# svenstaro/bvh

Hardware: AMD Instinct MI355X
Metric: Mrays/s (build+traverse) (higher is better)
Workload: dtype f32; 1 GPU; configs[1]: create_n_cubes(10000), 120000 triangles f32/3D, 1000000 create_ray rays per GPU; step = build_par+flatten+traverse; triangles=120000, rays_per_gpu=1000000, rays_total=1000000, scene_dist=single, flat_array=eager, parallelism=rays sharded x1

## Files before the change

bvh_amd/csrc/build.hip:

```cpp
#include "flatten_node.hpp"

namespace bvhgpu {

constexpr int MAXLV = 96;
constexpr int CTR_SMALL = 0;
constexpr int CTR_MID2 = 2;
constexpr int CTR_FLAGS = 4;
constexpr int CTR_TOPMASK = BUILD_CTR_TOPMASK;
constexpr uint32_t BUILD_FLAG_NONFINITE = 1u;
constexpr uint32_t BUILD_FLAG_PERSIST_GAVE_UP = BSTAT_UNFINISHED;
constexpr uint32_t BUILD_FLAG_EMPTY_SPLIT = 2u;
#ifndef BVH_MID_SMALL_MAXN
#define BVH_MID_SMALL_MAXN 768
#endif
#ifndef BVH_MID_SMALL_THREADS
#define BVH_MID_SMALL_THREADS 384
#endif
template <typename T> struct MidSmallScene {
    static constexpr int MAXN = BVH_MID_SMALL_MAXN;
    static constexpr int THREADS = BVH_MID_SMALL_THREADS;
    static constexpr int HANDOFF = SMALL_MAX;
};
#ifndef BVH_MID_LARGE_MAXN
#define BVH_MID_LARGE_MAXN 1536
#endif
#ifndef BVH_MID_LARGE_THREADS
#define BVH_MID_LARGE_THREADS 256
#endif
template <typename T> struct MidLargeScene {
    static constexpr int MAXN = sizeof(T) == 4 ? BVH_MID_LARGE_MAXN : BVH_MID_LARGE_MAXN * 2 / 3;
    static constexpr int THREADS = BVH_MID_LARGE_THREADS;
    static constexpr int HANDOFF = SMALL_MAX;
};
constexpr size_t MID_SCENE_SPLIT = 250000;
#ifndef BVH_STAT_REP
#define BVH_STAT_REP 8
#endif
constexpr int STAT_REP = BVH_STAT_REP;
constexpr int CTR_LEVEL0 = 16;
constexpr int CTR_XDIR = CTR_LEVEL0 + 2 * MAXLV;
static_assert((CTR_XDIR + 8 * 4) * 4 <= 1024, "the directory lives inside the counter page");
constexpr size_t ROOTKEY_OFF = 1024;
constexpr int PREP_MAX_WG = 1024;

__host__ __device__ inline int lvl_slot(int L) { return L < MAXLV - 2 ? L : (MAXLV - 2 + (L & 1)); }

template <typename T> struct ItemStats {
    typename Traits<T>::Key k[NUM_BUCKETS * STAT_KEYS];
    uint32_t cnt[NUM_BUCKETS];
    uint32_t _pad[2];
};

template <typename T> struct LevelArgs {
    Item<T>* item[2];
    uint4* tile_map[3];
    ItemStats<T>* stats[3];
    uint32_t* tile_cnt[3];
    uint8_t* bk[2];
    uint32_t slot_div, n_slots, n_tiles;
};

template <typename T> struct BuildArgs {
    LevelArgs<T> lv;
    uint32_t mid_max;
    const T* aabbs;
    const T* src;
    typename Traits<T>::Node* nodes;
    uint32_t* node_start;
    uint32_t* node_count;
    uint32_t* shape_node;
    uint16_t* node_slot;
    uint32_t* slot_entry;
    uint32_t n_slots;
    uint32_t* wslot_node;
    uint32_t* idx[2];
    uint8_t* bk;
    Item<T>* big[2];
    Item<T>* mid2;
    Item<T>* small;
    ItemStats<T>* stats[2];
    uint32_t* tile_item[2];
    uint32_t* tile_cnt;
    uint32_t* chunk_cnt[2];
    uint32_t n_chunks;
    FlattenArgs<T> fl;
    uint32_t fl_parts;
    uint32_t tile2;
    uint32_t* ctr;
    typename Traits<T>::Key* rootkeys;
    uint32_t prep_wgs;
    uint32_t n;
    unsigned long long* xbar;
};
constexpr int XBAR_WORDS = 8 * 32;

__device__ __forceinline__ bool key_is_min(int j) { return j < 3 || (j >= 6 && j < 9); }

template <typename T>
__device__ void push_item(const BuildArgs<T>& a, int next_level, uint32_t ni, uint32_t parent, uint32_t start,
                          uint32_t count, const T* A, const T* C, uint32_t heap, int lane);
template <typename T> __device__ void init_stats(ItemStats<T>* s, int lane);

template <typename T> __global__ __launch_bounds__(256) void k_prep(BuildArgs<T> a) {
    using Tr = Traits<T>;
    using Key = typename Tr::Key;
    __shared__ Key sk[STAT_KEYS];
    if (threadIdx.x < STAT_KEYS) sk[threadIdx.x] = key_is_min(threadIdx.x) ? Tr::KEY_POS_INF : Tr::KEY_NEG_INF;
    __syncthreads();
    T loc[STAT_KEYS];
#pragma unroll
    for (int j = 0; j < STAT_KEYS; j++) loc[j] = key_is_min(j) ? Tr::inf() : -Tr::inf();
    if (a.lv.tile_map[0]) {
        const uint32_t gt = blockIdx.x * blockDim.x + threadIdx.x, gs = gridDim.x * blockDim.x;
        for (uint32_t i = gt; i < 3u * a.lv.n_tiles; i += gs) a.lv.tile_map[i / a.lv.n_tiles][i % a.lv.n_tiles] = make_uint4(NONE, 0u, 0u, 0u);
        const uint32_t nc = a.lv.n_tiles * (uint32_t)NUM_BUCKETS;
        for (uint32_t i = gt; i < 3u * nc; i += gs) a.lv.tile_cnt[i / nc][i % nc] = 0u;
    }
    if (a.lv.tile_map[0] && blockIdx.x == 0 && threadIdx.x < WAVE)
        for (int r = 0; r < STAT_REP; r++) init_stats<T>(&a.lv.stats[0][r], (int)threadIdx.x);
    if (a.xbar && blockIdx.x == 0)
        for (uint32_t i = threadIdx.x; i < (uint32_t)XBAR_WORDS; i += blockDim.x) a.xbar[i] = 0ull;
    if (a.chunk_cnt[0] && blockIdx.x == 1 % gridDim.x)
        for (uint32_t i = threadIdx.x; i < 2u * a.n_chunks * 2u * (uint32_t)NUM_BUCKETS; i += blockDim.x) a.chunk_cnt[0][i] = 0u;
    if (blockIdx.x == 0) {
        for (uint32_t i = threadIdx.x; i < a.n_slots; i += blockDim.x) a.slot_entry[i] = NONE;
        for (uint32_t i = threadIdx.x; i < WIDE_SLOTS; i += blockDim.x) a.wslot_node[i] = NONE;
    }
    const bool copy = a.src != a.aabbs;
    T* own = const_cast<T*>(a.aabbs);
    bool bad = false;
    for (uint32_t i = blockIdx.x * blockDim.x + threadIdx.x; i < a.n; i += gridDim.x * blockDim.x) {
        a.idx[0][i] = i;
        const T* b = a.src + 6 * (size_t)i;
        T bx[6];
#pragma unroll
        for (int k = 0; k < 6; k++) bx[k] = b[k];
#pragma unroll
        for (int k = 0; k < 6; k++) bad = bad || !(fabs(bx[k]) < Tr::inf());
        if (copy) {
#pragma unroll
            for (int k = 0; k < 6; k++) own[6 * (size_t)i + k] = bx[k];
        }
#pragma unroll
        for (int k = 0; k < 3; k++) {
            const T c = center1(bx[k], bx[3 + k]);
            loc[k] = join_min(loc[k], bx[k]);
            loc[3 + k] = join_max(loc[3 + k], bx[3 + k]);
            loc[6 + k] = join_min(loc[6 + k], c);
            loc[9 + k] = join_max(loc[9 + k], c);
        }
    }
    {
        const int lane = lane_id();
#pragma unroll
        for (int d = 32; d > 0; d >>= 1) {
            T u[STAT_KEYS];
#pragma unroll
            for (int j = 0; j < STAT_KEYS; j++) u[j] = lane_fetch(loc[j], (lane ^ d) << 2);
#pragma unroll
            for (int j = 0; j < STAT_KEYS; j++) loc[j] = key_is_min(j) ? join_min(loc[j], u[j]) : join_max(loc[j], u[j]);
        }
        if (lane == 0) {
#pragma unroll
            for (int j = 0; j < STAT_KEYS; j++) {
                if (key_is_min(j)) atomicMin(&sk[j], Tr::key(loc[j]));
                else atomicMax(&sk[j], Tr::key(loc[j]));
            }
        }
    }
    if (a.n > 1 && __any(bad) && lane_id() == 0) atomicOr(&a.ctr[CTR_FLAGS], BUILD_FLAG_NONFINITE);
    __syncthreads();
    if (threadIdx.x < STAT_KEYS) a.rootkeys[(size_t)blockIdx.x * STAT_KEYS + threadIdx.x] = sk[threadIdx.x];
}

template <typename T> __global__ __launch_bounds__(256) void k_root(BuildArgs<T> a, uint32_t prep_wgs, int fused) {
    using Tr = Traits<T>;
    using Key = typename Tr::Key;
    __shared__ Key sk[STAT_KEYS];
    if (threadIdx.x < STAT_KEYS) sk[threadIdx.x] = key_is_min(threadIdx.x) ? Tr::KEY_POS_INF : Tr::KEY_NEG_INF;
    __syncthreads();
    for (uint32_t e = threadIdx.x; e < prep_wgs * (uint32_t)STAT_KEYS; e += blockDim.x) {
        const Key v = a.rootkeys[e];
        const int j = (int)(e % (uint32_t)STAT_KEYS);
        if (key_is_min(j)) atomicMin(&sk[j], v);
        else atomicMax(&sk[j], v);
    }
    __syncthreads();
    if (threadIdx.x < WAVE) {
        T A[6], C[6];
#pragma unroll
        for (int k = 0; k < 6; k++) { A[k] = Tr::unkey(sk[k]); C[k] = Tr::unkey(sk[6 + k]); }
        uint32_t flags = a.ctr[CTR_FLAGS];
        if (a.n > 1) {
            bool ovf = false;
#pragma unroll
            for (int k = 0; k < 3; k++) ovf = ovf || !(fabs(C[3 + k] - C[k]) < Tr::inf());
            if (ovf) { flags |= BUILD_FLAG_NONFINITE; if (threadIdx.x == 0) atomicOr(&a.ctr[CTR_FLAGS], BUILD_FLAG_NONFINITE); }
        }
        if (flags & BUILD_FLAG_NONFINITE) return;
        if (fused && a.n > a.mid_max) {
            const int lane = (int)threadIdx.x;
            Item<T>* it = &a.lv.item[0][0];
            if (lane == 0) {
                it->ni = 0; it->parent = 0; it->start = 0; it->count = a.n; it->tile_base = 0; it->parity = 0; it->heap = 1u; it->_r1 = 0;
                a.ctr[CTR_LEVEL0] = 1u;
            }
            if (lane < 6) { it->A[lane] = A[lane]; it->C[lane] = C[lane]; }
            const uint32_t ntile = (a.n + TILE - 1) / TILE;
            for (uint32_t j = lane; j < ntile; j += WAVE) a.lv.tile_map[0][j] = make_uint4(0u, 0u, a.n, 0u);
            for (int r = 0; r < STAT_REP; r++) init_stats<T>(&a.lv.stats[0][r], lane);
        } else {
            push_item<T>(a, 0, 0u, 0u, 0u, a.n, A, C, 1u, (int)threadIdx.x);
        }
    }
}

template <typename T> __device__ void init_stats(ItemStats<T>* s, int lane) {
    using Tr = Traits<T>;
    for (int j = lane; j < NUM_BUCKETS * STAT_KEYS; j += WAVE)
        s->k[j] = key_is_min(j % STAT_KEYS) ? Tr::KEY_POS_INF : Tr::KEY_NEG_INF;
    if (lane < NUM_BUCKETS) s->cnt[lane] = 0;
}

template <typename T>
__device__ void push_item(const BuildArgs<T>& a, int next_level, uint32_t ni, uint32_t parent, uint32_t start,
                          uint32_t count, const T* A, const T* C, uint32_t heap, int lane) {
    const int nslot = lvl_slot(next_level);
    const int npar = next_level & 1;
    uint32_t slot = 0, tb = 0;
    const bool is_small = count <= (uint32_t)SMALL_MAX;
    const bool is_mid2 = !is_small && count <= a.mid_max;
    const uint32_t ntile = (count + a.tile2 - 1) / a.tile2;
// ... 497 lines not shown
#pragma unroll
        for (int k = 0; k < 6; k++) { la[k] = Tr::unkey(scratch[sp * 6 + k]); ra[k] = Tr::unkey(scratch[36 + (sp + 1) * 6 + k]); }
        const T sa_parent = surface_area(A);
        const T cl = (T)ln * surface_area(la);
        const T cr = (T)(total - ln) * surface_area(ra);
        const T num = cl + cr;
        cost = num / sa_parent;
    }
    T min_cost = Tr::inf();
    int best = -1;
#pragma unroll
    for (int sp = 0; sp < NUM_BUCKETS - 1; sp++) {
        const T c = lane_bcast_rt(cost, sp);
        const bool take = degen ? (sp == 0) : (c < min_cost);
        if (take) { min_cost = c; best = sp; }
    }
    uint32_t nl = 0;
#pragma unroll
    for (int b = 0; b < NUM_BUCKETS; b++) nl += (best < 0 ? b == 0 : b <= best) ? cnt[b] : 0u;
    if (lane < 6) {
        const int k = lane;
        const bool mn = k < 3;
        T al, ar, cl, cr;
        if (best < 0) {
            al = ar = cl = cr = mn ? Tr::inf() : -Tr::inf();
        } else {
            Key kl = mn ? Tr::KEY_POS_INF : Tr::KEY_NEG_INF, kr = kl;
#pragma unroll
            for (int b = 0; b < NUM_BUCKETS; b++) {
                const Key x = stk[b * STAT_KEYS + 6 + k];
                const Key jl = mn ? (x < kl ? x : kl) : (x > kl ? x : kl);
                const Key jr = mn ? (x < kr ? x : kr) : (x > kr ? x : kr);
                kl = b <= best ? jl : kl;
                kr = b <= best ? kr : jr;
            }
            al = Tr::unkey(scratch[best * 6 + k]);
            ar = Tr::unkey(scratch[36 + (best + 1) * 6 + k]);
            cl = Tr::unkey(kl); cr = Tr::unkey(kr);
        }
        out->AL[k] = al; out->AR[k] = ar; out->CL[k] = cl; out->CR[k] = cr;
    }
    if (lane == 0) { out->nl = nl; out->no_winner = best < 0 ? 1u : 0u; }
    __builtin_amdgcn_fence(__ATOMIC_RELEASE, "wavefront");
    __builtin_amdgcn_wave_barrier();
    __builtin_amdgcn_fence(__ATOMIC_ACQUIRE, "wavefront");
}

template <typename T> struct LevelChild {
    uint32_t start, count, kind, slot, tile0, ax, degen, half;
    T cmin, ext;
};
constexpr int LEVEL_TGT = 4;

template <typename T> __device__ __forceinline__ void level_child_derive(LevelChild<T>* c, const T* C, uint32_t start, uint32_t count,
                                                                          uint32_t mid_max, uint32_t slot_div) {
    c->start = start; c->count = count;
    c->kind = count <= (uint32_t)SMALL_MAX ? 0u : (count <= mid_max ? 1u : 3u);
    c->slot = start / slot_div;
    c->tile0 = start / (uint32_t)TILE + c->slot;
    const int ax = largest_axis(C);
    c->ax = (uint32_t)ax;
    c->cmin = C[ax];
    c->ext = C[3 + ax] - C[ax];
    c->degen = (c->ext < Traits<T>::eps()) ? 1u : 0u;
    c->half = count / 2;
}

#ifdef BVH_LEVEL_PROFILE
__device__ unsigned long long g_level_prof[2 * 8 * 1024];
#define LEVEL_STAMP(i) do { if ((L == BVH_LEVEL_PROFILE || L == BVH_LEVEL_PROFILE + 1) && threadIdx.x == 0 && blockIdx.x < 1024) \
        g_level_prof[8 * (blockIdx.x + 1024 * (L - BVH_LEVEL_PROFILE)) + (i)] = wall_clock64(); } while (0)
#else
#define LEVEL_STAMP(i) do { } while (0)
#endif
__device__ __forceinline__ uint32_t wave_sum_u32(uint32_t x) {
    int v = (int)x;
    v += __builtin_amdgcn_update_dpp(0, v, 0x111, 0xF, 0xF, true);
    v += __builtin_amdgcn_update_dpp(0, v, 0x112, 0xF, 0xF, true);
    v += __builtin_amdgcn_update_dpp(0, v, 0x114, 0xF, 0xF, true);
    v += __builtin_amdgcn_update_dpp(0, v, 0x118, 0xF, 0xF, true);
    return (uint32_t)(__builtin_amdgcn_readlane(v, 15) + __builtin_amdgcn_readlane(v, 31) + __builtin_amdgcn_readlane(v, 47) +
                      __builtin_amdgcn_readlane(v, 63));
}
constexpr int LEVEL_TC_REP = 4;
constexpr int LEVEL_PT = TILE / 256;

#ifndef BVH_LEVEL_THREADS
#define BVH_LEVEL_THREADS 256
#endif
#ifndef BVH_LEVEL_EARLY_DUTIES
#define BVH_LEVEL_EARLY_DUTIES 1
#endif
constexpr int LEVEL_THREADS = BVH_LEVEL_THREADS;
constexpr bool LEVEL_DEDICATED = LEVEL_THREADS > 256;
constexpr unsigned long long XCD_SPIN_TICKS = 200000ull;
template <typename T, bool ROOT, bool DEV = false> __global__ __launch_bounds__(LEVEL_THREADS) void k_level(BuildArgs<T> a, int L_first) {
    using Tr = Traits<T>;
    using Key = typename Tr::Key;
    static_assert(TILE % 256 == 0 && LEVEL_PT >= 1 && LEVEL_PT <= 4, "a tile is a whole number of 256-thread rounds");
    static_assert(!(ROOT && DEV), "the root is binned by a launch of its own");
    const LevelArgs<T>& v = a.lv;
    uint32_t wg_rank = blockIdx.x, wg_count = gridDim.x, g0 = 0u, g1 = v.n_tiles, s0 = 0u, s1 = v.n_slots;
    __shared__ uint32_t s_live, s_go;
    __shared__ unsigned long long s_word;
    uint32_t live_seen = 0;
    if constexpr (DEV) {
        const uint32_t grp = blockIdx.x & 7u;
        wg_rank = blockIdx.x >> 3; wg_count = gridDim.x >> 3;
        const uint32_t* xd = &a.ctr[CTR_XDIR + 4 * grp];
        const uint32_t kind = xd[0], start = xd[2], count = xd[3];
        if (kind != 3u || (a.ctr[CTR_FLAGS] & BUILD_FLAG_NONFINITE)) return;
        const uint32_t sd = v.slot_div, end = start + count;
        g0 = start / (uint32_t)TILE + start / sd; g1 = end / (uint32_t)TILE + end / sd;
        s0 = start / sd; s1 = end / sd;
    }
    uint32_t* const live = &s_live;
  for (int L = L_first, round = 0; ; L++, round++) {
    if constexpr (DEV) {
        if (threadIdx.x == 0) s_live = 0u;
        __syncthreads();
    }
    const int bP = (L + 2) % 3, bC = L % 3, bN = (L + 1) % 3;
    const uint32_t* src = ROOT ? a.idx[0] : a.idx[(L + 1) & 1];
    uint32_t* dst = a.idx[L & 1];
    const uint8_t* bk_src = v.bk[(L + 1) & 1];
    uint8_t* bk_dst = v.bk[L & 1];
    const int lane = lane_id(), w = threadIdx.x >> 6;
    const bool shaper = !LEVEL_DEDICATED || w > 0;
    const int sw = LEVEL_DEDICATED ? w - 1 : w;
    const uint32_t stid = LEVEL_DEDICATED ? threadIdx.x - 64u : threadIdx.x;
    const unsigned long long lt = lanemask_lt();
    LEVEL_STAMP(0);
    uint4 tm_first = make_uint4(NONE, 0u, 0u, 0u);
    if (!ROOT && g0 + wg_rank < g1) tm_first = ldx4<DEV>(&v.tile_map[bP][g0 + wg_rank]);
    __shared__ Key s_rootk[STAT_KEYS];
    if (ROOT) {
        if (threadIdx.x < STAT_KEYS) s_rootk[threadIdx.x] = key_is_min(threadIdx.x) ? Tr::KEY_POS_INF : Tr::KEY_NEG_INF;
        __syncthreads();
        for (uint32_t e = threadIdx.x; e < a.prep_wgs * (uint32_t)STAT_KEYS; e += LEVEL_THREADS) {
            const Key x = a.rootkeys[e];
            const int j = (int)(e % (uint32_t)STAT_KEYS);
            if (key_is_min(j)) atomicMin(&s_rootk[j], x);
            else atomicMax(&s_rootk[j], x);
        }
        __syncthreads();
        bool bad = (a.ctr[CTR_FLAGS] & BUILD_FLAG_NONFINITE) != 0u;
#pragma unroll
        for (int k = 0; k < 3; k++) bad = bad || !(fabs(Tr::unkey(s_rootk[9 + k]) - Tr::unkey(s_rootk[6 + k])) < Tr::inf());
        if (bad) {
            if (blockIdx.x == 0 && threadIdx.x == 0) atomicOr(&a.ctr[CTR_FLAGS], BUILD_FLAG_NONFINITE);
            return;
        }
        const uint32_t root_tiles = (a.n + TILE - 1) / TILE;
        if (blockIdx.x == 0) {
            Item<T>* it = &v.item[0][0];
            if (threadIdx.x == 0) {
                it->ni = 0; it->parent = 0; it->start = 0; it->count = a.n; it->tile_base = 0; it->parity = 0; it->heap = 1u; it->_r1 = 0;
                a.ctr[CTR_LEVEL0] = 1u;
            }
            if (threadIdx.x < 6) { it->A[threadIdx.x] = Tr::unkey(s_rootk[threadIdx.x]); it->C[threadIdx.x] = Tr::unkey(s_rootk[6 + threadIdx.x]); }
            for (uint32_t j = threadIdx.x; j < root_tiles; j += LEVEL_THREADS) v.tile_map[0][j] = make_uint4(0u, 0u, a.n, 0u);
        }
        if (blockIdx.x < root_tiles) tm_first = make_uint4(0u, 0u, a.n, 0u);
    }

    {
        const uint32_t gt = wg_rank * (uint32_t)LEVEL_THREADS + threadIdx.x, gs = wg_count * (uint32_t)LEVEL_THREADS;
        for (uint32_t i = g0 + gt; i < g1; i += gs) {
            if constexpr (DEV) stx<true>(&v.tile_map[bN][i].x, NONE);
            else v.tile_map[bN][i] = make_uint4(NONE, 0u, 0u, 0u);
        }
        for (uint32_t i = g0 * (uint32_t)NUM_BUCKETS + gt; i < g1 * (uint32_t)NUM_BUCKETS; i += gs) stx<DEV>(&v.tile_cnt[bN][i], 0u);
        constexpr uint32_t NK = NUM_BUCKETS * STAT_KEYS;
        const uint32_t e0 = s0 * (uint32_t)STAT_REP, e1 = s1 * (uint32_t)STAT_REP;
        for (uint32_t i = e0 * NK + gt; i < e1 * NK; i += gs) {
            const uint32_t e = i / NK, j = i % NK;
            stx<DEV>(&v.stats[bN][e].k[j], key_is_min((int)(j % STAT_KEYS)) ? Tr::KEY_POS_INF : Tr::KEY_NEG_INF);
        }
        for (uint32_t i = e0 * (uint32_t)NUM_BUCKETS + gt; i < e1 * (uint32_t)NUM_BUCKETS; i += gs) stx<DEV>(&v.stats[bN][i / NUM_BUCKETS].cnt[i % NUM_BUCKETS], 0u);
    }

    __shared__ Key sk[2][BIN_REP][NUM_BUCKETS * STAT_KEYS];
    __shared__ uint32_t sc[2][BIN_REP][NUM_BUCKETS];
    __shared__ uint32_t tcnt[LEVEL_TC_REP][NUM_BUCKETS][LEVEL_TGT][NUM_BUCKETS];
    __shared__ uint32_t run0[NUM_BUCKETS], wsum[4][NUM_BUCKETS], wcnt[4][LEVEL_PT][NUM_BUCKETS];
    __shared__ LevelChild<T> ch[2];
    __shared__ LevelSel<T> sel;
    __shared__ ItemStats<T> s_merged;
    __shared__ Key s_sah[72];
    const int rp = (int)(stid & (BIN_REP - 1)), rt = (int)(stid & (LEVEL_TC_REP - 1));

    for (uint32_t g = g0 + wg_rank; g < g1; g += wg_count) {
        const uint4 tm = g == g0 + wg_rank ? tm_first : (ROOT ? make_uint4(g < (a.n + TILE - 1) / TILE ? 0u : NONE, 0u, a.n, 0u) : ldx4<DEV>(&v.tile_map[bP][g]));
        const uint32_t slotP = tm.x;
        if (slotP == NONE) continue;
        LEVEL_STAMP(1);
        const uint32_t start = tm.y, count = tm.z;
        const Item<T>* P = &v.item[ROOT ? 0 : ((L + 1) & 1)][slotP];
        const uint32_t tile0P = start / (uint32_t)TILE + slotP;
        const uint32_t tl = g - tile0P, ntl = (count + TILE - 1) / TILE;
        const uint32_t p0 = start + tl * TILE;
        const uint32_t pend = min(start + count, p0 + (uint32_t)TILE);

        Key rk[2][STAT_REP];
        uint32_t rc[STAT_REP];
        T PA[6], PC[6];
        uint32_t P_ni = 0, P_heap = 0, P_parent = 0;
        if (!ROOT && w == 0) {
            const ItemStats<T>* rep = &v.stats[bP][(size_t)slotP * STAT_REP];
#pragma unroll
            for (int h = 0; h < 2; h++) {
                const int j = lane + 64 * h;
#pragma unroll
                for (int r = 0; r < STAT_REP; r++) rk[h][r] = j < NUM_BUCKETS * STAT_KEYS ? ldx<DEV>(&rep[r].k[j]) : (Key)0;
            }
#pragma unroll
            for (int r = 0; r < STAT_REP; r++) rc[r] = lane < NUM_BUCKETS ? ldx<DEV>(&rep[r].cnt[lane]) : 0u;
#pragma unroll
            for (int k = 0; k < 6; k++) { PA[k] = ldx<DEV>(&P->A[k]); PC[k] = ldx<DEV>(&P->C[k]); }
            if (tl == 0) { P_ni = ldx<DEV>(&P->ni); P_heap = ldx<DEV>(&P->heap); P_parent = ldx<DEV>(&P->parent); }
        }
        uint32_t sh[LEVEL_PT];
        int bo[LEVEL_PT];
        T bx[LEVEL_PT][6];
#pragma unroll
        for (int u = 0; u < LEVEL_PT; u++) {
            const uint32_t p = p0 + (uint32_t)u * 256u + stid;
            const bool valid = shaper && p < pend;
            sh[u] = valid ? ldx<DEV>(&src[p]) : NONE;
            bo[u] = !valid ? 7 : (ROOT ? 0 : (int)ldx<DEV>(&bk_src[p]));
        }
        constexpr int TCV = 2;
        constexpr int NCT = LEVEL_THREADS - 64;
        const uint32_t ctid = threadIdx.x - 64u;
        uint32_t tcv[TCV][NUM_BUCKETS];
        const uint32_t* tc = v.tile_cnt[bP] + (size_t)tile0P * NUM_BUCKETS;
        if (!ROOT) {
#pragma unroll
            for (int i = 0; i < TCV; i++) {
                const uint32_t j = ctid + (uint32_t)NCT * (uint32_t)i;
#pragma unroll
                for (int b = 0; b < NUM_BUCKETS; b++) tcv[i][b] = (w > 0 && j < ntl) ? ldx<DEV>(&tc[(size_t)j * NUM_BUCKETS + b]) : 0u;
            }
        }
        auto tile0_duties = [&](const uint32_t nl) {
            const uint32_t ni = P_ni, heap = P_heap;
            const uint32_t li = ni + 1;
            const uint32_t ri = li + (2 * nl - 1);
            if (sel.no_winner && lane == 0) atomicOr(&a.ctr[CTR_FLAGS], BUILD_FLAG_EMPTY_SPLIT);
            if (lane == 0) {
                typename Tr::Node* nd = &a.nodes[ni];
#pragma unroll
                for (int k = 0; k < 3; k++) {
                    nd->l_min[k] = sel.AL[k]; nd->l_max[k] = sel.AL[3 + k];
                    nd->r_min[k] = sel.AR[k]; nd->r_max[k] = sel.AR[3 + k];
                }
                nd->parent = P_parent; nd->l = li; nd->r = ri; nd->shape = NONE;
                a.node_start[ni] = start;
                a.node_count[ni] = count;
                a.node_slot[ni] = (uint16_t)heap;
                if (heap < 16u) atomicOr(&a.ctr[CTR_TOPMASK], 1u << heap);
            }
            const uint32_t mykind = ch[lane & 1].kind;
            uint32_t cqs[2] = {0u, 0u};
            if (ch[0].kind != 3u || ch[1].kind != 3u) {
                uint32_t qslot = 0;
                if (lane < 2) {
                    if (mykind == 0u) qslot = atomicAdd(&a.ctr[CTR_SMALL], 1u);
                    else if (mykind == 1u) qslot = atomicAdd(&a.ctr[CTR_MID2], 1u);
                }
                cqs[0] = __shfl(qslot, 0); cqs[1] = __shfl(qslot, 1);
            }
            if (lane < 2 && mykind == 3u) atomicAdd(&a.ctr[CTR_LEVEL0 + 2 * lvl_slot(L)], 1u);
#pragma unroll
            for (int side = 0; side < 2; side++) {
                const LevelChild<T>& c = ch[side];
                const uint32_t cq = cqs[side];
                Item<T>* it = c.kind == 0u ? &a.small[cq] : (c.kind == 1u ? &a.mid2[cq] : &v.item[L & 1][c.slot]);
                if (lane == 0) {
                    stx<DEV>(&it->ni, side ? ri : li); stx<DEV>(&it->parent, ni); stx<DEV>(&it->start, c.start); stx<DEV>(&it->count, c.count);
                    stx<DEV>(&it->tile_base, c.tile0); stx<DEV>(&it->parity, (uint32_t)(L & 1)); stx<DEV>(&it->heap, heap_child(heap, (uint32_t)side)); stx<DEV>(&it->_r1, 0u);
                    const uint32_t hc = heap_child(heap, (uint32_t)side);
                    if (hc >= 8u && hc < 16u) {
                        uint32_t* xd = &a.ctr[CTR_XDIR + 4 * (hc - 8u)];
                        xd[0] = c.kind; xd[1] = c.slot; xd[2] = c.start; xd[3] = c.count;
                    }
                    if (DEV && c.kind == 3u) atomicAdd(live, 1u);
                }
                if (lane < 6) { stx<DEV>(&it->A[lane], side ? sel.AR[lane] : sel.AL[lane]); stx<DEV>(&it->C[lane], side ? sel.CR[lane] : sel.CL[lane]); }
                if (c.kind == 3u) {
                    const uint32_t cnt_t = (c.count + TILE - 1) / TILE;
                    for (uint32_t j = lane; j < cnt_t; j += WAVE) stx4<DEV>(&v.tile_map[bC][c.tile0 + j], make_uint4(c.slot, c.start, c.count, 0u));
                }
            }
                };
        if (ROOT) {
            if (threadIdx.x == 0) {
                T C[6];
#pragma unroll
                for (int k = 0; k < 6; k++) C[k] = Tr::unkey(s_rootk[6 + k]);
                level_child_derive<T>(&ch[0], C, start, count, a.mid_max, v.slot_div);
                ch[1].start = start + count; ch[1].count = 0; ch[1].kind = 0; ch[1].slot = 0; ch[1].tile0 = 0;
                sel.nl = count; sel.no_winner = 0;
            }
            if (threadIdx.x < NUM_BUCKETS) run0[threadIdx.x] = 0;
        } else if (w == 0) {
#pragma unroll
            for (int h = 0; h < 2; h++) {
                const int j = lane + 64 * h;
                if (j < NUM_BUCKETS * STAT_KEYS) {
                    const bool mn = key_is_min(j % STAT_KEYS);
                    Key x = rk[h][0];
#pragma unroll
                    for (int r = 1; r < STAT_REP; r++) { const Key u = rk[h][r]; x = mn ? (u < x ? u : x) : (u > x ? u : x); }
                    s_merged.k[j] = x;
                }
            }
            if (lane < NUM_BUCKETS) {
                uint32_t c = 0;
#pragma unroll
                for (int r = 0; r < STAT_REP; r++) c += rc[r];
                s_merged.cnt[lane] = c;
            }
            const int ax = largest_axis(PC);
            const bool degen = (PC[3 + ax] - PC[ax]) < Tr::eps();
            __builtin_amdgcn_fence(__ATOMIC_RELEASE, "wavefront");
            __builtin_amdgcn_wave_barrier();
            __builtin_amdgcn_fence(__ATOMIC_ACQUIRE, "wavefront");
            LEVEL_STAMP(7);
            sah_select_wave<T>(s_merged.k, s_merged.cnt, PA, degen, &sel, s_sah, lane);
#ifdef BVH_LEVEL_PROFILE
            LEVEL_STAMP(3);
#endif
            if (lane < 2) {
                const uint32_t nl = sel.nl;
                T CC[6];
#pragma unroll
                for (int k = 0; k < 6; k++) CC[k] = lane ? sel.CR[k] : sel.CL[k];
                level_child_derive<T>(&ch[lane], CC, lane ? start + nl : start, lane ? count - nl : nl, a.mid_max, v.slot_div);
            }
            if (BVH_LEVEL_EARLY_DUTIES && tl == 0) {
                __builtin_amdgcn_fence(__ATOMIC_RELEASE, "wavefront");
                __builtin_amdgcn_wave_barrier();
                __builtin_amdgcn_fence(__ATOMIC_ACQUIRE, "wavefront");
                tile0_duties(sel.nl);
            }
        } else {
            constexpr int NT3 = LEVEL_THREADS - 64;
            const int t3 = (int)threadIdx.x - 64;
            for (int j = t3; j < 2 * BIN_REP * NUM_BUCKETS * STAT_KEYS; j += NT3)
                (&sk[0][0][0])[j] = key_is_min(j % STAT_KEYS) ? Tr::KEY_POS_INF : Tr::KEY_NEG_INF;
            for (int j = t3; j < 2 * BIN_REP * NUM_BUCKETS; j += NT3) (&sc[0][0][0])[j] = 0u;
            for (int j = t3; j < LEVEL_TC_REP * NUM_BUCKETS * LEVEL_TGT * NUM_BUCKETS; j += NT3) (&tcnt[0][0][0][0])[j] = 0u;
        }
        if (ROOT) {
            for (int j = threadIdx.x; j < 2 * BIN_REP * NUM_BUCKETS * STAT_KEYS; j += LEVEL_THREADS)
                (&sk[0][0][0])[j] = key_is_min(j % STAT_KEYS) ? Tr::KEY_POS_INF : Tr::KEY_NEG_INF;
            for (int j = threadIdx.x; j < 2 * BIN_REP * NUM_BUCKETS; j += LEVEL_THREADS) (&sc[0][0][0])[j] = 0u;
            for (int j = threadIdx.x; j < LEVEL_TC_REP * NUM_BUCKETS * LEVEL_TGT * NUM_BUCKETS; j += LEVEL_THREADS) (&tcnt[0][0][0][0])[j] = 0u;
        }
#pragma unroll
        for (int u = 0; u < LEVEL_PT; u++) {
            if (sh[u] != NONE) {
                const T* bp = a.aabbs + 6 * (size_t)sh[u];
#pragma unroll
                for (int k = 0; k < 6; k++) bx[u][k] = bp[k];
            } else {
#pragma unroll
                for (int k = 0; k < 6; k++) bx[u][k] = (T)0;
            }
        }
        if (!ROOT && w > 0) {
            uint32_t before[NUM_BUCKETS], all[NUM_BUCKETS];
#pragma unroll
            for (int b = 0; b < NUM_BUCKETS; b++) { before[b] = 0; all[b] = 0; }
#pragma unroll
            for (int i = 0; i < TCV; i++) {
                const uint32_t j = ctid + (uint32_t)NCT * (uint32_t)i;
#pragma unroll
                for (int b = 0; b < NUM_BUCKETS; b++) { all[b] += tcv[i][b]; before[b] += j < tl ? tcv[i][b] : 0u; }
            }
            for (uint32_t j = ctid + (uint32_t)NCT * TCV; j < ntl; j += NCT) {
#pragma unroll
                for (int b = 0; b < NUM_BUCKETS; b++) {
                    const uint32_t x = ldx<DEV>(&tc[(size_t)j * NUM_BUCKETS + b]);
                    all[b] += x;
                    before[b] += j < tl ? x : 0u;
                }
            }
            uint32_t acc = 0;
#pragma unroll
            for (int b = 0; b < NUM_BUCKETS; b++) {
                const uint32_t mine = wave_sum_u32(acc + before[b]);
                acc += all[b];
                if (lane == 0) wsum[w - 1][b] = mine;
            }
        }
        uint32_t rank[LEVEL_PT];
#pragma unroll
        for (int u = 0; u < LEVEL_PT; u++) rank[u] = 0;
        if (!ROOT && shaper) {
#pragma unroll
            for (int u = 0; u < LEVEL_PT; u++) {
                rank[u] = 0;
#pragma unroll
                for (int bb = 0; bb < NUM_BUCKETS; bb++) {
                    const unsigned long long m = __ballot(bo[u] == bb);
                    if (bo[u] == bb) rank[u] = (uint32_t)__popcll(m & lt);
                    if (lane == 0) wcnt[sw][u][bb] = (uint32_t)__popcll(m);
                }
            }
        }
        LEVEL_STAMP(2);
        lds_barrier();
        if (!ROOT && threadIdx.x < NUM_BUCKETS) {
            uint32_t r0 = 0;
#pragma unroll
            for (int ww = 0; ww < LEVEL_THREADS / 64 - 1; ww++) r0 += wsum[ww][threadIdx.x];
            run0[threadIdx.x] = r0;
        }
        if (!ROOT) lds_barrier();
        const uint32_t nl = sel.nl;
#pragma unroll
        for (int u = 0; u < LEVEL_PT; u++) {
            if (sh[u] == NONE) continue;
            const uint32_t p = p0 + (uint32_t)u * 256u + stid;
            const int b = bo[u];
            uint32_t off;
            if (ROOT) {
                off = p - start;
            } else {
                off = run0[b] + rank[u];
                for (int uu = 0; uu < u; uu++) off += wcnt[0][uu][b] + wcnt[1][uu][b] + wcnt[2][uu][b] + wcnt[3][uu][b];
                for (int ww = 0; ww < sw; ww++) off += wcnt[ww][u][b];
                stx<DEV>(&dst[start + off], sh[u]);
            }
            const int side = off >= nl ? 1 : 0;
            const LevelChild<T>& c = ch[side];
            if (c.kind == 3u) {
                T cen[3];
#pragma unroll
                for (int k = 0; k < 3; k++) cen[k] = center1(bx[u][k], bx[u][3 + k]);
                const uint32_t q = start + off;
                int nb;
                if (c.degen) nb = (q - c.start) < c.half ? 0 : 1;
                else nb = bucket_of(cen[c.ax], c.cmin, c.ext);
                stx<DEV>(&bk_dst[q], (uint8_t)nb);
                Key* kk = &sk[side][rp][nb * STAT_KEYS];
#pragma unroll
                for (int k = 0; k < 3; k++) {
                    atomicMin(&kk[k], Tr::key(bx[u][k]));
                    atomicMax(&kk[3 + k], Tr::key(bx[u][3 + k]));
                    const Key kc = Tr::key(cen[k]);
                    atomicMin(&kk[6 + k], kc);
                    atomicMax(&kk[9 + k], kc);
                }
                atomicAdd(&sc[side][rp][nb], 1u);
                const uint32_t off_first = ROOT ? (p0 - start) : run0[b];
                const int side_first = off_first >= nl ? 1 : 0;
                const uint32_t kt = (q - c.start) / (uint32_t)TILE;
                const uint32_t kt_first = (start + off_first - ch[side_first].start) / (uint32_t)TILE;
                const uint32_t tgt = side != side_first ? 2u + kt : kt - kt_first;
                atomicAdd(&tcnt[rt][b][tgt][nb], 1u);
            }
        }
        lds_barrier();
        LEVEL_STAMP(4);
        for (int e = threadIdx.x; e < 2 * NUM_BUCKETS * STAT_KEYS; e += LEVEL_THREADS) {
            const int side = e / (NUM_BUCKETS * STAT_KEYS), j = e % (NUM_BUCKETS * STAT_KEYS);
            if (ch[side].kind != 3u) continue;
            uint32_t cn = 0;
#pragma unroll
            for (int r = 0; r < BIN_REP; r++) cn += sc[side][r][j / STAT_KEYS];
            if (!cn) continue;
            Key x = sk[side][0][j];
            const bool mn = key_is_min(j % STAT_KEYS);
#pragma unroll
            for (int r = 1; r < BIN_REP; r++) { const Key u = sk[side][r][j]; x = mn ? (u < x ? u : x) : (u > x ? u : x); }
// ... 808 lines not shown
        tile_grid = (int)std::min<size_t>(n / level_tile<T>(t) + max_big + 2, 2048);
        sel_grid = (int)std::min<size_t>((max_big + 3) / 4, 1024);
        mid2_grid = (int)std::min<size_t>(max_mid2, (size_t)t->ctx->n_cu * 4);
        small_grid = (int)std::min<size_t>((n + 3) / 4, (size_t)t->ctx->n_cu * 8);
        level_grid = (int)std::min<size_t>(LevelLayout<T>(n, mid_max).n_tiles, 2048);
    }
};

template <typename T> static void run_level(bvhgpu_tree* t, const BuildArgs<T>& a, const BuildGrid<T>& g, int L) {
    hipStream_t st = t->ctx->stream;
    if (level_fused<T>(t)) {
        if (L == 0) hipLaunchKernelGGL((k_level<T, true>), dim3(g.level_grid), dim3(LEVEL_THREADS), 0, st, a, 0);
        hipLaunchKernelGGL((k_level<T, false>), dim3(g.level_grid), dim3(LEVEL_THREADS), 0, st, a, L + 1);
        return;
    }
    hipLaunchKernelGGL(k_bin<T>, dim3(g.tile_grid), dim3(256), 0, st, a, L);
    hipLaunchKernelGGL(k_split<T>, dim3(g.sel_grid + g.tile_grid), dim3(256), 0, st, a, L, (uint32_t)g.sel_grid);
}
template <typename T> static void run_lower_tiers(bvhgpu_tree* t, const BuildArgs<T>& a, const BuildGrid<T>& g, uint32_t mid2_done,
                                                  uint32_t small_done) {
    hipStream_t st = t->ctx->stream;
    if (t->n > (size_t)SMALL_MAX) {
        if (t->n <= MID_SCENE_SPLIT) hipLaunchKernelGGL((k_mid<T, MidSmallScene<T>>), dim3(g.mid2_grid), dim3(MidSmallScene<T>::THREADS), 0, st, a, mid2_done);
        else hipLaunchKernelGGL((k_mid<T, MidLargeScene<T>>), dim3(g.mid2_grid), dim3(MidLargeScene<T>::THREADS), 0, st, a, mid2_done);
    }
    if (a.fl_parts != 0u) hipLaunchKernelGGL((k_small<T, true>), dim3(g.small_grid), dim3(256), 0, st, a, small_done);
    else hipLaunchKernelGGL((k_small<T, false>), dim3(g.small_grid), dim3(256), 0, st, a, small_done);
}

template <typename T> void build_enqueue(bvhgpu_tree* t, const T* aabbs_dev, size_t n, bool flatten_after, bool redo) {
    using Tr = Traits<T>;
    using Key = typename Tr::Key;
    bvhgpu_ctx* ctx = t->ctx;
    hipStream_t st = ctx->stream;
    join_flat(t);
    t->built = false; t->flattened = false; t->lazy_flat = false; t->pending_build = false; t->exact_only = false; t->pending_recv = false;
    t->pend_persist = false;
    if (!redo) t->gen++;
    if (n != t->n) { t->has_tris = false; t->has_spheres = false; }
    t->n = n; t->n_nodes = n ? 2 * n - 1 : 0;
    t->n_flat = n >= 2 ? 3 * n - 2 : n;
    t->n_trav = n >= 2 ? 2 * n - 2 : n;
    t->levels = 0;
    if (n == 0) { t->built = true; t->flattened = flatten_after; return; }

    const size_t MID_MAX = n <= MID_SCENE_SPLIT ? (size_t)MidSmallScene<T>::MAXN : (size_t)MidLargeScene<T>::MAXN;
    const BuildGrid<T> g(t, MID_MAX);
    t->aabbs.reserve(n * 6 * sizeof(T));
    if (t->nodes.reserve(t->n_nodes * sizeof(typename Tr::Node))) BVH_HIP(hipMemsetAsync(t->nodes.p, 0, t->nodes.cap, st));
    if (t->node_start.reserve(t->n_nodes * 4)) BVH_HIP(hipMemsetAsync(t->node_start.p, 0, t->node_start.cap, st));
    if (t->node_count.reserve(t->n_nodes * 4)) BVH_HIP(hipMemsetAsync(t->node_count.p, 0, t->node_count.cap, st));
    t->shape_node.reserve(n * 4);
    if (t->node_slot.reserve(t->n_nodes * 2)) BVH_HIP(hipMemsetAsync(t->node_slot.p, 0xFF, t->node_slot.cap, st));
    t->slot_entry.reserve(TopCfg<T>::SLOTS * 4);
    t->wslot_node.reserve(WIDE_SLOTS * 4);
    t->idx[0].reserve(n * 4);
    t->idx[1].reserve(n * 4);
    t->bk.reserve(2 * n);
    if (level_fused<T>(t) && n > (size_t)MID_MAX) t->lvbuf.reserve(LevelLayout<T>(n, MID_MAX).bytes);
    const int persist_knob = ctx->tune[BVHGPU_TUNE_BUILD_LEVEL_PERSIST];
    if (t->persist_broken && persist_knob != 0 && !redo && t->persist_retry_in > 0 && --t->persist_retry_in == 0) t->persist_broken = false;
    const bool persist = persist_knob != 0 && !t->persist_broken && level_fused<T>(t) && n >= 32 * (MID_MAX + 1);
    if (persist) t->xbar.reserve(XBAR_WORDS * sizeof(unsigned long long));
    for (int i = 0; i < 2; i++) {
        t->big[i].reserve(g.max_big * sizeof(Item<T>));
        t->stats[i].reserve(g.max_big * STAT_REP * sizeof(ItemStats<T>));
        t->tile_item[i].reserve(g.max_tiles * 4);
    }
    t->mid2.reserve(g.max_mid2 * sizeof(Item<T>));
    t->small.reserve((n + 1) * sizeof(Item<T>));
    t->tile_cnt.reserve(g.max_tiles * NUM_BUCKETS * 4);
    if (!level_fused<T>(t)) t->chunk_cnt.reserve((g.max_tiles / CHUNK_TILES + 2) * 2 * 2 * NUM_BUCKETS * 4);
    if (t->ctr.reserve(ROOTKEY_OFF + (size_t)PREP_MAX_WG * STAT_KEYS * sizeof(Key))) t->ctr_ready = false;
    if (!t->pin) BVH_HIP(hipHostMalloc(&t->pin, ROOTKEY_OFF, hipHostMallocDefault));

    BuildArgs<T> a = make_args<T>(t, aabbs_dev);
    if (!t->ctr_ready) hipLaunchKernelGGL(k_init<T>, dim3(1), dim3(256), 0, st, a);
    t->ctr_ready = false;
#ifndef BVH_PREP_PER_WG
#define BVH_PREP_PER_WG 1024
#endif
    const int prep_grid = (int)std::min<size_t>((n + BVH_PREP_PER_WG - 1) / BVH_PREP_PER_WG, (size_t)PREP_MAX_WG);
    a.prep_wgs = (uint32_t)prep_grid;
    hipLaunchKernelGGL(k_prep<T>, dim3(prep_grid), dim3(256), 0, st, a);
    if (!(level_fused<T>(t) && n > (size_t)MID_MAX)) hipLaunchKernelGGL(k_root<T>, dim3(1), dim3(256), 0, st, a, (uint32_t)prep_grid, 0);

    int level = 0;
    if (n > (size_t)MID_MAX) {
        int fixed = 1;
        for (size_t m = n; m > (size_t)MID_MAX; m = (m + 1) / 2) fixed++;
        if (t->hint_levels > 0 && t->hint_n == n) fixed = t->hint_levels;
        if (fixed > MAXLV - 4) fixed = MAXLV - 4;
        if (persist) {
            for (; level < 3; level++) run_level<T>(t, a, g, level);
            const int nx = persist_knob >= 8 ? std::min(persist_knob, 64) : 32;
            hipLaunchKernelGGL((k_level<T, false, true>), dim3(8 * nx), dim3(LEVEL_THREADS), 0, st, a, 4);
            t->pend_persist = true;
            fixed = level;
        }
        for (; level < fixed; level++) {
            run_level<T>(t, a, g, level);
            if (level == 3 && ctx->tune[BVHGPU_TUNE_WIDE_EARLY_ITEMS] != 0 && !t->pend_persist) {
                if (!t->ev_top) BVH_HIP(hipEventCreateWithFlags(&t->ev_top, hipEventDisableTiming));
                BVH_HIP(hipEventRecord(t->ev_top, st));
                t->ev_top_gen = t->gen;
            }
        }
    }
    uint32_t inline_parts = 0;
    if (flatten_after && n >= 2 && sizeof(T) == 4 && ctx->tune[BVHGPU_TUNE_FLATTEN_INLINE] != 0) {
        const FlattenPlan p = flatten_plan<T>(t, ctx->tune[BVHGPU_TUNE_FLATTEN_LAZY] != 0);
        if (p.with_wide) {
            inline_parts = (uint32_t)(p.parts & (FLATTEN_FLAT | FLATTEN_WIDE));
            a.fl = flatten_args<T>(t, p.with_wide, p.with_guide); a.fl_parts = inline_parts;
        }
    }
    run_lower_tiers<T>(t, a, g, 0u, 0u);
    t->bstat.reserve(64);
    if (flatten_after && n >= 1)
        flatten_tree<T>(t, a.ctr, reinterpret_cast<uint32_t*>(t->pin), (uint32_t)(ROOTKEY_OFF / 4), t->bstat.as<uint32_t>(), (uint32_t)CTR_FLAGS,
                        (n > (size_t)MID_MAX && !t->pend_persist) ? (uint32_t)(CTR_LEVEL0 + 2 * lvl_slot(level)) : (uint32_t)CTR_FLAGS,
                        ctx->tune[BVHGPU_TUNE_FLATTEN_LAZY] != 0, inline_parts);
    else hipLaunchKernelGGL(k_publish_build<T>, dim3(1), dim3(256), 0, st, a, reinterpret_cast<uint32_t*>(t->pin));
    t->ctr_ready = true;
    t->pending_build = true; t->pend_level = level; t->pend_flatten = flatten_after;
}

template <typename T> void build_finalize(bvhgpu_tree* t) {
    if (!t->pending_build) return;
    t->pending_build = false;
    bvhgpu_ctx* ctx = t->ctx;
    hipStream_t st = ctx->stream;
    join_flat(t);
    BVH_HIP(hipStreamSynchronize(st));
    BVH_HIP(hipGetLastError());
    const size_t n = t->n;
    const size_t MID_MAX = n <= MID_SCENE_SPLIT ? (size_t)MidSmallScene<T>::MAXN : (size_t)MidLargeScene<T>::MAXN;
    uint32_t* pin = reinterpret_cast<uint32_t*>(t->pin);
    if (pin[CTR_FLAGS] & BUILD_FLAG_NONFINITE) {
        t->flattened = false;
        t->failed_gen = t->gen; t->failed_what = Fail::NonFinite;
        throw HipFail{hipErrorInvalidValue, nullptr, __LINE__, Fail::NonFinite};
    }
    if (t->pend_persist && (pin[CTR_FLAGS] & BUILD_FLAG_PERSIST_GAVE_UP)) {
        t->persist_broken = true;
        t->persist_retry_in = 64;
        const bool fl = t->pend_flatten;
        build_enqueue<T>(t, static_cast<const T*>(nullptr), n, fl, true);
        build_finalize<T>(t);
        t->redone_gen = t->gen;
        return;
    }
    int level = t->pend_persist ? MAXLV - 3 : t->pend_level;
    if (n > (size_t)MID_MAX && !t->pend_persist && pin[CTR_LEVEL0 + 2 * lvl_slot(level)] != 0) {
        const BuildGrid<T> g(t, MID_MAX);
        const BuildArgs<T> a = make_args<T>(t, nullptr);
        BVH_HIP(hipMemcpyAsync(a.ctr, t->pin, ROOTKEY_OFF, hipMemcpyHostToDevice, st));
        t->ctr_ready = false;
        uint32_t mid2_done = pin[CTR_MID2], small_done = pin[CTR_SMALL];
        while (true) {
            if (level + 1 >= MAXLV - 2)
                BVH_HIP(hipMemsetAsync(a.ctr + CTR_LEVEL0 + 2 * lvl_slot(level + 1), 0, 8, st));
            run_level<T>(t, a, g, level);
            level++;
            BVH_HIP(hipMemcpyAsync(t->pin, a.ctr, ROOTKEY_OFF, hipMemcpyDeviceToHost, st));
            BVH_HIP(hipStreamSynchronize(st));
            if (pin[CTR_LEVEL0 + 2 * lvl_slot(level)] == 0) break;
// ... 43 lines not shown
```

Baseline: 3021 Mrays/s.

## Unroll prep loop and hoist level box gathers ahead of tile0 duties

In k_prep, the per-element loop is unrolled by four so all loads are issued before the reductions and stores, and launch dims become compile-time constants. The tile_map and tile_cnt indexing is rewritten with pointer selects. In k_level, the AABB gather is issued earlier (inside tile0 duties and before the prefix sums), and empty asm constraints place the waits later so memory latency overlaps other work. The root level uses p directly instead of loading src[p], which assumes the root index is the identity. Invalid slots now read box 0 instead of zeros, which adds register pressure and relies on those slots being ignored downstream.

Result: no change. 3073 Mrays/s, median of 4 (+1.7%).

```diff
diff --git a/bvh_amd/csrc/build.hip b/bvh_amd/csrc/build.hip
--- a/bvh_amd/csrc/build.hip
+++ b/bvh_amd/csrc/build.hip
@@ -101,7 +101,8 @@
                           uint32_t count, const T* A, const T* C, uint32_t heap, int lane);
 template <typename T> __device__ void init_stats(ItemStats<T>* s, int lane);
 
-template <typename T> __global__ __launch_bounds__(256) void k_prep(BuildArgs<T> a) {
+constexpr uint32_t PREP_THREADS = 256;
+template <typename T> __global__ __launch_bounds__(PREP_THREADS) void k_prep(BuildArgs<T> a) {
     using Tr = Traits<T>;
     using Key = typename Tr::Key;
     __shared__ Key sk[STAT_KEYS];
@@ -110,44 +111,67 @@
     T loc[STAT_KEYS];
 #pragma unroll
     for (int j = 0; j < STAT_KEYS; j++) loc[j] = key_is_min(j) ? Tr::inf() : -Tr::inf();
+    const uint32_t gt = blockIdx.x * PREP_THREADS + threadIdx.x, gs = a.prep_wgs * PREP_THREADS;
     if (a.lv.tile_map[0]) {
-        const uint32_t gt = blockIdx.x * blockDim.x + threadIdx.x, gs = gridDim.x * blockDim.x;
-        for (uint32_t i = gt; i < 3u * a.lv.n_tiles; i += gs) a.lv.tile_map[i / a.lv.n_tiles][i % a.lv.n_tiles] = make_uint4(NONE, 0u, 0u, 0u);
+        uint4* const tm0 = a.lv.tile_map[0]; uint4* const tm1 = a.lv.tile_map[1]; uint4* const tm2 = a.lv.tile_map[2];
+        for (uint32_t i = gt; i < 3u * a.lv.n_tiles; i += gs) {
+            const uint32_t r = i / a.lv.n_tiles;
+            (r == 0u ? tm0 : (r == 1u ? tm1 : tm2))[i % a.lv.n_tiles] = make_uint4(NONE, 0u, 0u, 0u);
+        }
         const uint32_t nc = a.lv.n_tiles * (uint32_t)NUM_BUCKETS;
-        for (uint32_t i = gt; i < 3u * nc; i += gs) a.lv.tile_cnt[i / nc][i % nc] = 0u;
+        uint32_t* const tc0 = a.lv.tile_cnt[0]; uint32_t* const tc1 = a.lv.tile_cnt[1]; uint32_t* const tc2 = a.lv.tile_cnt[2];
+        for (uint32_t i = gt; i < 3u * nc; i += gs) {
+            const uint32_t r = i / nc;
+            (r == 0u ? tc0 : (r == 1u ? tc1 : tc2))[i % nc] = 0u;
+        }
     }
     if (a.lv.tile_map[0] && blockIdx.x == 0 && threadIdx.x < WAVE)
         for (int r = 0; r < STAT_REP; r++) init_stats<T>(&a.lv.stats[0][r], (int)threadIdx.x);
     if (a.xbar && blockIdx.x == 0)
-        for (uint32_t i = threadIdx.x; i < (uint32_t)XBAR_WORDS; i += blockDim.x) a.xbar[i] = 0ull;
-    if (a.chunk_cnt[0] && blockIdx.x == 1 % gridDim.x)
-        for (uint32_t i = threadIdx.x; i < 2u * a.n_chunks * 2u * (uint32_t)NUM_BUCKETS; i += blockDim.x) a.chunk_cnt[0][i] = 0u;
+        for (uint32_t i = threadIdx.x; i < (uint32_t)XBAR_WORDS; i += PREP_THREADS) a.xbar[i] = 0ull;
+    if (a.chunk_cnt[0] && blockIdx.x == 1u % a.prep_wgs)
+        for (uint32_t i = threadIdx.x; i < 2u * a.n_chunks * 2u * (uint32_t)NUM_BUCKETS; i += PREP_THREADS) a.chunk_cnt[0][i] = 0u;
     if (blockIdx.x == 0) {
-        for (uint32_t i = threadIdx.x; i < a.n_slots; i += blockDim.x) a.slot_entry[i] = NONE;
-        for (uint32_t i = threadIdx.x; i < WIDE_SLOTS; i += blockDim.x) a.wslot_node[i] = NONE;
+        for (uint32_t i = threadIdx.x; i < a.n_slots; i += PREP_THREADS) a.slot_entry[i] = NONE;
+        for (uint32_t i = threadIdx.x; i < WIDE_SLOTS; i += PREP_THREADS) a.wslot_node[i] = NONE;
     }
     const bool copy = a.src != a.aabbs;
     T* own = const_cast<T*>(a.aabbs);
     bool bad = false;
-    for (uint32_t i = blockIdx.x * blockDim.x + threadIdx.x; i < a.n; i += gridDim.x * blockDim.x) {
-        a.idx[0][i] = i;
-        const T* b = a.src + 6 * (size_t)i;
-        T bx[6];
-#pragma unroll
-        for (int k = 0; k < 6; k++) bx[k] = b[k];
-#pragma unroll
-        for (int k = 0; k < 6; k++) bad = bad || !(fabs(bx[k]) < Tr::inf());
-        if (copy) {
-#pragma unroll
-            for (int k = 0; k < 6; k++) own[6 * (size_t)i + k] = bx[k];
-        }
-#pragma unroll
-        for (int k = 0; k < 3; k++) {
-            const T c = center1(bx[k], bx[3 + k]);
-            loc[k] = join_min(loc[k], bx[k]);
-            loc[3 + k] = join_max(loc[3 + k], bx[3 + k]);
-            loc[6 + k] = join_min(loc[6 + k], c);
-            loc[9 + k] = join_max(loc[9 + k], c);
+    constexpr int PREP_UNROLL = 4;
+    for (uint32_t i0 = gt; i0 < a.n; i0 += (uint32_t)PREP_UNROLL * gs) {
+        T bx[PREP_UNROLL][6];
+        uint32_t iu[PREP_UNROLL];
+#pragma unroll
+        for (int u = 0; u < PREP_UNROLL; u++) {
+            const uint32_t iw = i0 + (uint32_t)u * gs;
+            iu[u] = iw < a.n ? iw : NONE;
+            const T* b = a.src + 6 * (size_t)(iw < a.n ? iw : a.n - 1u);
+#pragma unroll
+            for (int k = 0; k < 6; k++) bx[u][k] = b[k];
+        }
+#pragma unroll
+        for (int u = 0; u < PREP_UNROLL; u++) {
+#pragma unroll
+            for (int k = 0; k < 6; k++) bad = bad || !(fabs(bx[u][k]) < Tr::inf());
+#pragma unroll
+            for (int k = 0; k < 3; k++) {
+                const T c = center1(bx[u][k], bx[u][3 + k]);
+                loc[k] = join_min(loc[k], bx[u][k]);
+                loc[3 + k] = join_max(loc[3 + k], bx[u][3 + k]);
+                loc[6 + k] = join_min(loc[6 + k], c);
+                loc[9 + k] = join_max(loc[9 + k], c);
+            }
+        }
+#pragma unroll
+        for (int u = 0; u < PREP_UNROLL; u++) {
+            if (iu[u] == NONE) continue;
+            const uint32_t i = iu[u];
+            a.idx[0][i] = i;
+            if (copy) {
+#pragma unroll
+                for (int k = 0; k < 6; k++) own[6 * (size_t)i + k] = bx[u][k];
+            }
         }
     }
     {
@@ -811,6 +835,7 @@
     return (uint32_t)(__builtin_amdgcn_readlane(v, 15) + __builtin_amdgcn_readlane(v, 31) + __builtin_amdgcn_readlane(v, 47) +
                       __builtin_amdgcn_readlane(v, 63));
 }
+template <typename U> __device__ __forceinline__ void vm_arrived(U& x) { asm volatile("" : "+v"(x)); }
 constexpr int LEVEL_TC_REP = 4;
 constexpr int LEVEL_PT = TILE / 256;
 
@@ -956,7 +981,7 @@
         for (int u = 0; u < LEVEL_PT; u++) {
             const uint32_t p = p0 + (uint32_t)u * 256u + stid;
             const bool valid = shaper && p < pend;
-            sh[u] = valid ? ldx<DEV>(&src[p]) : NONE;
+            sh[u] = valid ? (ROOT ? p : ldx<DEV>(&src[p])) : NONE;
             bo[u] = !valid ? 7 : (ROOT ? 0 : (int)ldx<DEV>(&bk_src[p]));
         }
         constexpr int TCV = 2;
@@ -972,6 +997,18 @@
                 for (int b = 0; b < NUM_BUCKETS; b++) tcv[i][b] = (w > 0 && j < ntl) ? ldx<DEV>(&tc[(size_t)j * NUM_BUCKETS + b]) : 0u;
             }
         }
+        if (!ROOT) {
+#pragma unroll
+            for (int u = 0; u < LEVEL_PT; u++) { vm_arrived(sh[u]); vm_arrived(bo[u]); }
+        }
+        auto gather_boxes = [&]() {
+#pragma unroll
+            for (int u = 0; u < LEVEL_PT; u++) {
+                const T* bp = a.aabbs + 6 * (size_t)(sh[u] != NONE ? sh[u] : 0u);
+#pragma unroll
+                for (int k = 0; k < 6; k++) bx[u][k] = bp[k];
+            }
+        };
         auto tile0_duties = [&](const uint32_t nl) {
             const uint32_t ni = P_ni, heap = P_heap;
             const uint32_t li = ni + 1;
@@ -1053,6 +1090,7 @@
             }
             const int ax = largest_axis(PC);
             const bool degen = (PC[3 + ax] - PC[ax]) < Tr::eps();
+            gather_boxes();
             __builtin_amdgcn_fence(__ATOMIC_RELEASE, "wavefront");
             __builtin_amdgcn_wave_barrier();
             __builtin_amdgcn_fence(__ATOMIC_ACQUIRE, "wavefront");
@@ -1068,6 +1106,11 @@
                 for (int k = 0; k < 6; k++) CC[k] = lane ? sel.CR[k] : sel.CL[k];
                 level_child_derive<T>(&ch[lane], CC, lane ? start + nl : start, lane ? count - nl : nl, a.mid_max, v.slot_div);
             }
+#pragma unroll
+            for (int u = 0; u < LEVEL_PT; u++) {
+#pragma unroll
+                for (int k = 0; k < 6; k++) vm_arrived(bx[u][k]);
+            }
             if (BVH_LEVEL_EARLY_DUTIES && tl == 0) {
                 __builtin_amdgcn_fence(__ATOMIC_RELEASE, "wavefront");
                 __builtin_amdgcn_wave_barrier();
@@ -1088,17 +1131,7 @@
             for (int j = threadIdx.x; j < 2 * BIN_REP * NUM_BUCKETS; j += LEVEL_THREADS) (&sc[0][0][0])[j] = 0u;
             for (int j = threadIdx.x; j < LEVEL_TC_REP * NUM_BUCKETS * LEVEL_TGT * NUM_BUCKETS; j += LEVEL_THREADS) (&tcnt[0][0][0][0])[j] = 0u;
         }
-#pragma unroll
-        for (int u = 0; u < LEVEL_PT; u++) {
-            if (sh[u] != NONE) {
-                const T* bp = a.aabbs + 6 * (size_t)sh[u];
-#pragma unroll
-                for (int k = 0; k < 6; k++) bx[u][k] = bp[k];
-            } else {
-#pragma unroll
-                for (int k = 0; k < 6; k++) bx[u][k] = (T)0;
-            }
-        }
+        if (ROOT || w > 0) gather_boxes();
         if (!ROOT && w > 0) {
             uint32_t before[NUM_BUCKETS], all[NUM_BUCKETS];
 #pragma unroll
@@ -1123,6 +1156,11 @@
                 const uint32_t mine = wave_sum_u32(acc + before[b]);
                 acc += all[b];
                 if (lane == 0) wsum[w - 1][b] = mine;
+            }
+#pragma unroll
+            for (int u = 0; u < LEVEL_PT; u++) {
+#pragma unroll
+                for (int k = 0; k < 6; k++) vm_arrived(bx[u][k]);
             }
         }
         uint32_t rank[LEVEL_PT];
@@ -2097,7 +2135,7 @@
 #endif
     const int prep_grid = (int)std::min<size_t>((n + BVH_PREP_PER_WG - 1) / BVH_PREP_PER_WG, (size_t)PREP_MAX_WG);
     a.prep_wgs = (uint32_t)prep_grid;
-    hipLaunchKernelGGL(k_prep<T>, dim3(prep_grid), dim3(256), 0, st, a);
+    hipLaunchKernelGGL(k_prep<T>, dim3(prep_grid), dim3(PREP_THREADS), 0, st, a);
     if (!(level_fused<T>(t) && n > (size_t)MID_MAX)) hipLaunchKernelGGL(k_root<T>, dim3(1), dim3(256), 0, st, a, (uint32_t)prep_grid, 0);
 
     int level = 0;
```
